# eliotwang/SageAttention

Measured on AMD Instinct MI355X. Metric: attention fwd TFLOPS at head_dim=128 seqlen=8192 (INT8 QK^T + FP16 PV, quantizers included), higher is better.
Workload: dtype int8+fp16; 1 GPU; c3: qk_int8_pv_fp16 (B,H,N,D)=(4,32,8192,128) causal=False qk_quant_gran=per_thread; global_batch=4, seq_len=8192, head_dim=128, heads=32, parallelism=single

## Files before the change

sageattention_amd/_build.py:

```python
import os
import subprocess
import sys

HERE = os.path.dirname(os.path.abspath(__file__))
CSRC = os.path.join(HERE, "csrc")
LIB = os.path.join(HERE, "libsageattn_hip.so")
HIPCC = os.environ.get("HIPCC", "/opt/rocm/bin/hipcc")
ARCH = "gfx950"

SOURCES = [
    ("sage_quant.hip", ["-ffp-contract=off"]),
    ("sage_attn.hip", ["-fno-slp-vectorize", "-ffp-contract=off"]),
    ("sage_fp8.hip", []),
    ("sage_misc.hip", []),
    ("sage_op.hip", []),
    ("sage_sparge.hip", []),
]
COMMON = ["-O3", "-std=c++17", "-fPIC", f"--offload-arch={ARCH}", "-Wall", "-Wno-unused-function", "-Wno-inline-asm",
          "-Rpass-analysis=kernel-resource-usage"]


def _check_no_scratch(src, compiler_output):
    import re
    name = None
    for line in compiler_output.splitlines():
        m = re.search(r"Function Name: (\S+)", line)
        if m:
            name = m.group(1)
        m = re.search(r"ScratchSize \[bytes/lane\]: (\d+)", line)
        if m and int(m.group(1)) != 0:
            raise RuntimeError(f"{src}: kernel {name} uses {m.group(1)} bytes/lane of scratch (register spill)")


def _check_occupancy(src, compiler_output):
    import re
    name = None
    for line in compiler_output.splitlines():
        m = re.search(r"Function Name: (\S+)", line)
        if m:
            name = m.group(1)
        m = re.search(r" VGPRs: (\d+)", line)
        guarded = name and (re.search(r"attn_i8_kernelILi64ELi4E(Lb[01]E){4}Lb0EEE", name) or
                            re.search(r"attn_i8_blocksparse_kernelILi64E(Lb[01]E){3}EE", name))
        if m and guarded and int(m.group(1)) > 168:
            raise RuntimeError(f"{src}: kernel {name} uses {m.group(1)} VGPRs (> 168: two waves per SIMD instead of three)")


def _check_m0_private(obj):
    import glob
    import re
    import shutil
    import tempfile
    objdump = os.path.join(os.path.dirname(os.path.dirname(HIPCC)), "lib", "llvm", "bin", "llvm-objdump")
    if not os.path.exists(objdump):
        objdump = "/opt/rocm/lib/llvm/bin/llvm-objdump"
    tmp = tempfile.mkdtemp(prefix="sage_m0_")
    try:
        local = os.path.join(tmp, "o.o")
        shutil.copy(obj, local)
        subprocess.run([objdump, "--offloading", local], stdout=subprocess.DEVNULL, stderr=subprocess.DEVNULL, check=True)
        dev = glob.glob(local + ".*" + ARCH)
        if not dev:
            raise RuntimeError(f"{obj}: no {ARCH} code object found")
        dis = subprocess.run([objdump, "-d", dev[0]], stdout=subprocess.PIPE, text=True, check=True).stdout
        bad = [l.strip() for l in dis.splitlines() if re.search(r"\bm0\b", l) and not re.search(r"s_mov_b32 m0, s\d+", l)]
        if bad:
            raise RuntimeError(f"{obj}: M0 is used outside lds_dma16:\n" + "\n".join(bad[:5]))
    finally:
        shutil.rmtree(tmp, ignore_errors=True)


def _digest(*parts) -> str:
    import hashlib
    h = hashlib.sha256()
    for part in parts:
        h.update(part if isinstance(part, bytes) else str(part).encode())
        h.update(b"\0")
    return h.hexdigest()


def _read(path) -> bytes:
    with open(path, "rb") as f:
        return f.read()


def _stamp_ok(target, key) -> bool:
    try:
        return os.path.exists(target) and _read(target + ".stamp").decode().strip() == key
    except OSError:
        return False


def _write_stamp(target, key):
    with open(target + ".stamp", "w") as f:
        f.write(key + "\n")


def build(force: bool = False, verbose: bool = False) -> str:
    hdrs = [os.path.join(CSRC, f) for f in sorted(os.listdir(CSRC)) if f.endswith(".h")]
    hdrs.append(os.path.join(HERE, "..", "include", "sageattn_hip.h"))
    hdr_key = _digest(*[_read(h) for h in hdrs])
    keys = {src: _digest(HIPCC, ARCH, " ".join(COMMON + extra), _read(os.path.join(CSRC, src)), hdr_key)
            for src, extra in SOURCES}
    lib_key = _digest(*[keys[src] for src, _ in SOURCES])
    if not force and _stamp_ok(LIB, lib_key):
        return LIB
    objs = []
    procs = []
    for src, extra in SOURCES:
        s = os.path.join(CSRC, src)
        o = os.path.join(CSRC, src.replace(".hip", ".o"))
        objs.append(o)
        if force or not _stamp_ok(o, keys[src]):
            cmd = [HIPCC] + COMMON + extra + ["-c", s, "-o", o]
            if verbose:
                print(" ".join(cmd), flush=True)
            procs.append((src, o, subprocess.Popen(cmd, stdout=subprocess.PIPE, stderr=subprocess.STDOUT, text=True)))
    for src, o, pr in procs:
        out, _ = pr.communicate()
        if pr.returncode != 0:
            raise RuntimeError(f"hipcc failed on {src}:\n{out}")
        try:
            _check_no_scratch(src, out)
            _check_occupancy(src, out)
        except RuntimeError:
            os.remove(o)
            raise
        _write_stamp(o, keys[src])
        if verbose:
            print("\n".join(l for l in out.splitlines() if "remark:" not in l))
    _check_m0_private(os.path.join(CSRC, "sage_attn.o"))
    cmd = [HIPCC, "-shared", "-fPIC", f"--offload-arch={ARCH}", "-o", LIB] + objs
    r = subprocess.run(cmd, stdout=subprocess.PIPE, stderr=subprocess.STDOUT, text=True)
    if r.returncode != 0:
        raise RuntimeError(f"link failed:\n{r.stdout}")
    _write_stamp(LIB, lib_key)
    return LIB


if __name__ == "__main__":
    print(build(force="--force" in sys.argv, verbose=True))
```

sageattention_amd/csrc/sage_quant.hip:

```cpp
#include "sage_entry.h"
#include "sage_fp8_kernels.h"

namespace sage {

constexpr int KMEAN_ROWS = 256;
__host__ __device__ __forceinline__ int kmean_chunk_rows(int N) {
  const int c256 = (N + KMEAN_ROWS - 1) / KMEAN_ROWS;
  return KMEAN_ROWS * ((c256 + 15) / 16 > 0 ? (c256 + 15) / 16 : 1);
}

template <int D, bool BF16>
__device__ __forceinline__ void k_mean_partial_body(const uint16_t* __restrict__ k, int64_t sb, int64_t sh, int64_t sn, int N,
                                                    float* __restrict__ part, int S, int s, int h, int b, int H,
                                                    float (*red)[D + 1]) {
  constexpr int TPR = D / 8;
  constexpr int RPP = 256 / TPR;
  const int tr = threadIdx.x / TPR, tc = threadIdx.x % TPR;
  const uint16_t* base = k + b * sb + h * sh + tc * 8;
  float acc[8] = {0, 0, 0, 0, 0, 0, 0, 0};
  const int rows = kmean_chunk_rows(N);
  const int r0 = s * rows;
  if (r0 + rows <= N) {
#pragma unroll 8
    for (int i = 0; i < rows / RPP; ++i) {
      const uint4 u = *reinterpret_cast<const uint4*>(base + (int64_t)(r0 + i * RPP + tr) * sn);
      float f[8];
      unpack8<BF16>(u, f);
#pragma unroll
      for (int j = 0; j < 8; ++j) acc[j] += f[j];
    }
  } else {
#pragma unroll 4
    for (int i = 0; i < rows / RPP; ++i) {
      const int row = r0 + i * RPP + tr;
      if (row < N) {
        const uint4 u = *reinterpret_cast<const uint4*>(base + (int64_t)row * sn);
        float f[8];
        unpack8<BF16>(u, f);
#pragma unroll
        for (int j = 0; j < 8; ++j) acc[j] += f[j];
      }
    }
  }
#pragma unroll
  for (int j = 0; j < 8; ++j) red[tr][tc * 8 + j] = acc[j];
  __syncthreads();
  if (threadIdx.x < D) {
    float sum = 0.f;
    for (int r = 0; r < RPP; ++r) sum += red[r][threadIdx.x];
    part[(((int64_t)b * H + h) * S + s) * D + threadIdx.x] = sum;
  }
}

template <int D, bool BF16>
__global__ __launch_bounds__(256) void k_mean_partial_kernel(const uint16_t* __restrict__ k, int64_t sb, int64_t sh,
                                                             int64_t sn, int N, float* __restrict__ part, int S) {
  __shared__ float red[256 / (D / 8)][D + 1];
  k_mean_partial_body<D, BF16>(k, sb, sh, sn, N, part, S, blockIdx.x, blockIdx.y, blockIdx.z, gridDim.y, red);
}

template <bool BF16>
__global__ void k_mean_final_kernel(const float* __restrict__ part, int S, int D, int N, uint16_t* __restrict__ km) {
  const int64_t bh = blockIdx.x;
  const int d = threadIdx.x;
  if (d >= D) return;
  float sum = 0.f;
  for (int s0 = 0; s0 < S; s0 += 8) {
    float v[8];
#pragma unroll
    for (int u = 0; u < 8; ++u) v[u] = part[(bh * S + min(s0 + u, S - 1)) * D + d];
#pragma unroll
    for (int u = 0; u < 8; ++u)
      if (s0 + u < S) sum += v[u];
  }
  km[bh * D + d] = f32_to_elem_bits<BF16>(sum / (float)N);
}


template <int CTRL>
__device__ __forceinline__ float dpp_lane(float x) {
  return __builtin_bit_cast(float, __builtin_amdgcn_update_dpp(0, __builtin_bit_cast(int, x), CTRL, 0xf, 0xf, false));
}
template <int TPR>
__device__ __forceinline__ float row_lanes_max(float a) {
  static_assert(TPR == 8 || TPR == 16, "a row is 8 or 16 lanes");
  a = fmaxf(a, dpp_lane<0xB1>(a));
  a = fmaxf(a, dpp_lane<0x4E>(a));
  a = fmaxf(a, dpp_lane<0x141>(a));
  if constexpr (TPR == 16) a = fmaxf(a, dpp_lane<0x140>(a));
  return a;
}

__device__ __forceinline__ int group_of_row(int lr, int gran, int is_key, int warp_shift) {
  if (gran == SAGE_GRAN_PER_BLOCK) return 0;
  const int w = lr >> warp_shift;
  if (gran == SAGE_GRAN_PER_WARP) return w;
  return is_key ? w * 4 + ((lr & 7) >> 1) : w * 8 + (lr & 7);
}

template <int D, int BLK>
struct QuantGeom {
  static constexpr int TPR = D / 8;
  static constexpr int RPP = 256 / TPR;
  static constexpr int NP = BLK / RPP;
  static_assert(NP >= 1, "block too small");
};

template <int D, int BLK>
__device__ __forceinline__ void quant_load_rows(const uint16_t* xbase, const int64_t xsn, const int blk, const int N_,
                                                uint4 (&raw)[QuantGeom<D, BLK>::NP]) {
  using G = QuantGeom<D, BLK>;
  int tid = threadIdx.x;
  asm volatile("" : "+v"(tid));
  const int tr = tid / G::TPR;
#pragma unroll
  for (int i = 0; i < G::NP; ++i) {
    const int row = blk * BLK + i * G::RPP + tr;
    raw[i] = make_uint4(0, 0, 0, 0);
    if (row < N_) raw[i] = *reinterpret_cast<const uint4*>(xbase + (int64_t)row * xsn);
  }
}

template <int D, bool BF16>
__device__ __forceinline__ uint4 quant_mean_bits(const QuantParams& p, const int h, const int b, const int H, const bool store_km,
                                                 float (*mpart)[D]) {
  constexpr int TPR = D / 8;
  const int tr = threadIdx.x / TPR, tc = threadIdx.x % TPR;
  if (p.mean_part && tr < p.S) {
    const float* pp = p.mean_part + (((int64_t)b * H + h) * p.S + tr) * D + tc * 8;
    *reinterpret_cast<float4*>(&mpart[tr][tc * 8]) = *reinterpret_cast<const float4*>(pp);
    *reinterpret_cast<float4*>(&mpart[tr][tc * 8 + 4]) = *reinterpret_cast<const float4*>(pp + 4);
  }
  __syncthreads();
  uint4 mbits = make_uint4(0u, 0u, 0u, 0u);
  if (p.mean_part) {
    if (tr == 0) {
      float sum[8] = {0, 0, 0, 0, 0, 0, 0, 0};
      for (int s_ = 0; s_ < p.S; ++s_) {
        const float4 a = *reinterpret_cast<const float4*>(&mpart[s_][tc * 8]), c = *reinterpret_cast<const float4*>(&mpart[s_][tc * 8 + 4]);
        sum[0] += a.x; sum[1] += a.y; sum[2] += a.z; sum[3] += a.w; sum[4] += c.x; sum[5] += c.y; sum[6] += c.z; sum[7] += c.w;
      }
      uint32_t w[4];
#pragma unroll
      for (int j = 0; j < 8; ++j) {
        const uint16_t bits = f32_to_elem_bits<BF16>(sum[j] / (float)p.N);
        if (j & 1) w[j >> 1] |= (uint32_t)bits << 16; else w[j >> 1] = bits;
      }
      mbits = make_uint4(w[0], w[1], w[2], w[3]);
      *reinterpret_cast<uint4*>(&mpart[0][tc * 8]) = mbits;
      if (store_km) *reinterpret_cast<uint4*>(p.km_out + ((int64_t)b * H + h) * D + tc * 8) = mbits;
    }
    __syncthreads();
    mbits = *reinterpret_cast<const uint4*>(&mpart[0][tc * 8]);
  } else if (p.mean) {
    mbits = *reinterpret_cast<const uint4*>(p.mean + ((int64_t)(p.cu ? 0 : b) * H + h) * D + tc * 8);
  }
  return mbits;
}

template <int D, int BLK, bool BF16, bool TRITON, typename AfterPhase1>
__device__ __forceinline__ void quant_block(const QuantParams& p, const int blk, const int h, const int b, const int H, const int N_,
                                            const int64_t o_boff, uint4 (&raw)[QuantGeom<D, BLK>::NP], const uint4 mbits,
                                            unsigned int* gmax, unsigned int* zero_next, AfterPhase1 after_phase1) {
  using G = QuantGeom<D, BLK>;
  constexpr int TPR = G::TPR, RPP = G::RPP, NP = G::NP;
  int tid = threadIdx.x;
  asm volatile("" : "+v"(tid));
  const int tr = tid / TPR, tc = tid % TPR;
  float xf[NP][8];
  float dvec[8];
  if (p.dot_vec) {
    const int Hk = H / p.dot_group;
    const uint4 ud = *reinterpret_cast<const uint4*>(p.dot_vec + ((int64_t)b * Hk + h / p.dot_group) * D + tc * 8);
    unpack8<BF16>(ud, dvec);
  }

  {
    float mean_f[8];
    if constexpr (!TRITON || BF16) unpack8<BF16>(mbits, mean_f);
#pragma unroll
    for (int i = 0; i < NP; ++i) {
      const int lr = i * RPP + tr;
      const int row = blk * BLK + lr;
      const bool valid = row < N_;
      if (p.dot_vec) {
        float xr[8];
        unpack8<BF16>(raw[i], xr);
        float dot = 0.f;
#pragma unroll
        for (int j = 0; j < 8; ++j) dot += xr[j] * dvec[j];
#pragma unroll
        for (int o = 1; o < TPR; o <<= 1) dot += __shfl_xor(dot, o);
        if (tc == 0 && valid) p.dot_out[((int64_t)b * H + h) * p.N + row] = dot;
      }
      if constexpr (TRITON && !BF16) {
        const uint32_t xw[4] = {raw[i].x, raw[i].y, raw[i].z, raw[i].w}, mw[4] = {mbits.x, mbits.y, mbits.z, mbits.w};
#pragma unroll
        for (int w = 0; w < 4; ++w) {
          const v2h d = __builtin_bit_cast(v2h, xw[w]) - __builtin_bit_cast(v2h, mw[w]);
          xf[i][2 * w] = (float)d[0];
          xf[i][2 * w + 1] = (float)d[1];
        }
      } else {
        unpack8<BF16>(raw[i], xf[i]);
#pragma unroll
        for (int j = 0; j < 8; ++j) {
          xf[i][j] = xf[i][j] - mean_f[j];
          if constexpr (TRITON) xf[i][j] = round_to_elem<BF16>(xf[i][j]);
        }
      }
      float amax = 0.f;
      const float mult_row = valid ? p.mult : 0.f;
#pragma unroll
      for (int j = 0; j < 8; ++j) {
        xf[i][j] = xf[i][j] * mult_row;
        amax = fmaxf(amax, fabsf(xf[i][j]));
      }
      amax = row_lanes_max<TPR>(amax);
      if (tc == 0) atomicMax(&gmax[group_of_row(lr, p.gran, p.is_key, p.warp_shift)], __float_as_uint(amax));
    }
  }
  after_phase1();
  __syncthreads();
  if (zero_next && threadIdx.x < 64) zero_next[threadIdx.x] = 0u;

  const int groups_per_blk = p.gran == SAGE_GRAN_PER_BLOCK ? 1
                             : p.gran == SAGE_GRAN_PER_WARP ? BLK >> p.warp_shift
                                                            : (BLK >> p.warp_shift) * (p.is_key ? 4 : 8);
  const float eps = (p.gran == SAGE_GRAN_PER_THREAD) ? 0.0000001f : 0.f;
  if (threadIdx.x < groups_per_blk) {
    const float a = __uint_as_float(gmax[threadIdx.x]);
    const float sc = TRITON ? a / 127.f + eps : fmaxf(a, 0.0000001f) / 127.f;
    p.scale[b * p.ss_b + h * p.ss_h + blk * p.ss_blk + threadIdx.x] = sc;
  }

  int8_t* obase = p.out + o_boff + h * p.osh + blk * p.o_blk + tc * 8;
#pragma unroll
  for (int i = 0; i < NP; ++i) {
    const int lr = i * RPP + tr;
    const int row = blk * BLK + lr;
    const float a = __uint_as_float(gmax[group_of_row(lr, p.gran, p.is_key, p.warp_shift)]);
    int q[8];
    if constexpr (TRITON) {
      const float sc = a / 127.f + eps;
      const float r = 1.0f / sc;
      bool near = false;
#pragma unroll
      for (int j = 0; j < 8; ++j) q[j] = round_half_away_fast(xf[i][j] * r, near);
      if (__builtin_amdgcn_ballot_w64(near || !(fabsf(r) < 3.0e38f)) != 0) {
#pragma unroll
        for (int j = 0; j < 8; ++j) {
          float y = xf[i][j] / sc;
          y = y + (y >= 0.f ? 0.5f : -0.5f);
          q[j] = min(max((int)y, -128), 127);
        }
      }
    } else {
      const float inv = 127.f / fmaxf(a, 0.0000001f);
#pragma unroll
      for (int j = 0; j < 8; ++j) q[j] = (int)rintf(xf[i][j] * inv);
    }
    const uint32_t w0 = pack_i8x4(q[0], q[1], q[2], q[3]), w1 = pack_i8x4(q[4], q[5], q[6], q[7]);
    if (row < N_) *reinterpret_cast<uint2*>(obase + (int64_t)lr * p.osn) = make_uint2(w0, w1);
  }
}

template <int D, int BLK, bool BF16, bool TRITON>
__device__ __forceinline__ void quant_qk_int8_body(const QuantParams& p, const int blk, const int h, const int b, const int H,
                                                   unsigned int* gmax, float (*mpart)[D]) {
  int N_ = p.N;
  int64_t x_boff = b * p.xsb, o_boff = b * p.osb;
  if (p.cu) {
    const int lo = p.cu[b];
    N_ = p.cu[b + 1] - lo;
    if (blk * BLK >= N_) return;
    x_boff = (int64_t)lo * p.xsn;
    o_boff = (int64_t)lo * p.osn;
  }
  if (threadIdx.x < 64) gmax[threadIdx.x] = 0u;
  uint4 raw[QuantGeom<D, BLK>::NP];
  quant_load_rows<D, BLK>(p.x + x_boff + h * p.xsh + (threadIdx.x % (D / 8)) * 8, p.xsn, blk, N_, raw);
  const uint4 mbits = quant_mean_bits<D, BF16>(p, h, b, H, blk == 0, mpart);
  quant_block<D, BLK, BF16, TRITON>(p, blk, h, b, H, N_, o_boff, raw, mbits, gmax, nullptr, [] {});
}

template <int D, int BLK, bool BF16, bool TRITON>
__global__ __launch_bounds__(256, BLK * D <= 64 * 128 ? 7 : 4) void quant_qk_int8_kernel(const QuantParams p) {
  __shared__ unsigned int gmax[64];
  __shared__ __attribute__((aligned(16))) float mpart[16][D];
  quant_qk_int8_body<D, BLK, BF16, TRITON>(p, blockIdx.x, blockIdx.y, blockIdx.z, gridDim.y, gmax, mpart);
}

template <int D, bool BF16, bool TRITON>
__device__ __forceinline__ void k_quant_stream_body(const QuantParams& p, const int per_wg, const int wg, const int h, const int b,
                                                    const int H, unsigned int (*gmax)[64], float (*mpart)[D]) {
  constexpr int BLK = 64;
  using G = QuantGeom<D, BLK>;
  const int nblk = (p.N + BLK - 1) / BLK;
  const int blk0 = wg * per_wg, blk1 = min(blk0 + per_wg, nblk);
  if (threadIdx.x < 192) (&gmax[0][0])[threadIdx.x] = 0u;
  const uint16_t* xbase = p.x + b * p.xsb + h * p.xsh + (threadIdx.x % G::TPR) * 8;
  const int64_t o_boff = b * p.osb;
  uint4 raw[G::NP];
  quant_load_rows<D, BLK>(xbase, p.xsn, blk0, p.N, raw);
  const uint4 mbits = quant_mean_bits<D, BF16>(p, h, b, H, wg == 0, mpart);
  int par = 0;
  for (int blk = blk0; blk < blk1; ++blk) {
    quant_block<D, BLK, BF16, TRITON>(p, blk, h, b, H, p.N, o_boff, raw, mbits, gmax[par], gmax[par == 0 ? 2 : par - 1], [&] {
      if (blk + 1 < blk1) quant_load_rows<D, BLK>(xbase, p.xsn, blk + 1, p.N, raw);
    });
    par = par == 2 ? 0 : par + 1;
  }
}

template <int D, bool BF16, bool TRITON>
__global__ __launch_bounds__(256, D == 64 ? 5 : 4) void k_quant_stream_kernel(const QuantParams p, const int per_wg) {
  __shared__ unsigned int gmax[3][64];
  __shared__ __attribute__((aligned(16))) float mpart[16][D];
  k_quant_stream_body<D, BF16, TRITON>(p, per_wg, blockIdx.x, blockIdx.y, blockIdx.z, gridDim.y, gmax, mpart);
}


template <int D, bool BF16>
__device__ __forceinline__ void v_amax_partial_body(const uint16_t* __restrict__ v, int64_t sb, int64_t sh, int64_t sn, int N,
                                                    float* __restrict__ part, int S, int s, int h, int b, int H,
                                                    float (*red)[D + 1]) {
  constexpr int TPR = D / 8, RPP = 256 / TPR;
  const int tr = threadIdx.x / TPR, tc = threadIdx.x % TPR;
  const uint16_t* base = v + b * sb + h * sh + tc * 8;
  float am[8] = {0, 0, 0, 0, 0, 0, 0, 0};
  const int rows = kmean_chunk_rows(N);
  if ((s + 1) * rows <= N) {
#pragma unroll 8
    for (int i = 0; i < rows / RPP; ++i) {
      float f[8];
      unpack8<BF16>(*reinterpret_cast<const uint4*>(base + (int64_t)(s * rows + i * RPP + tr) * sn), f);
#pragma unroll
      for (int j = 0; j < 8; ++j) am[j] = fmaxf(am[j], fabsf(f[j]));
    }
  } else {
#pragma unroll 4
    for (int i = 0; i < rows / RPP; ++i) {
      const int row = s * rows + i * RPP + tr;
      if (row < N) {
        float f[8];
        unpack8<BF16>(*reinterpret_cast<const uint4*>(base + (int64_t)row * sn), f);
#pragma unroll
        for (int j = 0; j < 8; ++j) am[j] = fmaxf(am[j], fabsf(f[j]));
      }
    }
  }
#pragma unroll
  for (int j = 0; j < 8; ++j) red[tr][tc * 8 + j] = am[j];
  __syncthreads();
  if (threadIdx.x < D) {
    float a = red[0][threadIdx.x];
    for (int r = 1; r < RPP; ++r) a = fmaxf(a, red[r][threadIdx.x]);
    part[(((int64_t)b * H + h) * S + s) * D + threadIdx.x] = a;
  }
}

template <int D, bool BF16>
__global__ __launch_bounds__(256) void kv_partial_kernel(const uint16_t* __restrict__ k, int64_t ksb, int64_t ksh, int64_t ksn,
                                                         const uint16_t* __restrict__ v, int64_t vsb, int64_t vsh, int64_t vsn,
                                                         int N, float* __restrict__ kpart, float* __restrict__ vpart, int S) {
  static_assert(KMEAN_ROWS == VQ_ROWS, "one chunk size for both tensors");
  __shared__ float red[256 / (D / 8)][D + 1];
  const int x = blockIdx.x;
  if (x < S) k_mean_partial_body<D, BF16>(k, ksb, ksh, ksn, N, kpart, S, x, blockIdx.y, blockIdx.z, gridDim.y, red);
  else v_amax_partial_body<D, BF16>(v, vsb, vsh, vsn, N, vpart, S, x - S, blockIdx.y, blockIdx.z, gridDim.y, red);
}

template <int D, bool BF16, bool TRITON>
__global__ __launch_bounds__(256, D == 64 ? 8 : 7) void kv_quant_kernel(const QuantParams p, const VPrepParams q, const int nblk_k) {
  using G = VQuantGeom<D>;
  __shared__ unsigned int gmax[64];
  __shared__ __attribute__((aligned(16))) float exch[16][D];
  __shared__ __attribute__((aligned(16))) uint32_t tile[G::BLKS * G::IMG];
  const int h = blockIdx.y, b = blockIdx.z, H = gridDim.y;
  if ((int)blockIdx.x < nblk_k) {
    quant_qk_int8_body<D, 64, BF16, TRITON>(p, blockIdx.x, h, b, H, gmax, exch);
    return;
  }
  const int bx = blockIdx.x - nblk_k;
  const int tg = threadIdx.x / G::TPR, tc = threadIdx.x % G::TPR;
  uint4 raw[4];
  v_quant_load<D>(q.v + b * q.sb + h * q.sh, q.sn, p.N, bx, raw);
  if (tg < p.S) {
    const float* pp = q.part + (((int64_t)b * H + h) * p.S + tg) * D + tc * 8;
    *reinterpret_cast<float4*>(&exch[tg][tc * 8]) = *reinterpret_cast<const float4*>(pp);
    *reinterpret_cast<float4*>(&exch[tg][tc * 8 + 4]) = *reinterpret_cast<const float4*>(pp + 4);
  }
  __syncthreads();
  if (tg == 0) {
    float rc[8], vs[8];
#pragma unroll
    for (int j = 0; j < 8; ++j) {
      float a = exch[0][tc * 8 + j];
      for (int s_ = 1; s_ < p.S; ++s_) a = fmaxf(a, exch[s_][tc * 8 + j]);
      rc[j] = q.scale_max / a;
      vs[j] = a / q.scale_max;
    }
#pragma unroll
    for (int j = 0; j < 8; ++j) exch[0][tc * 8 + j] = rc[j];
    if (bx == 0) {
      float* o = q.v_scale + ((int64_t)b * H + h) * D + tc * 8;
      *reinterpret_cast<float4*>(o) = make_float4(vs[0], vs[1], vs[2], vs[3]);
      *reinterpret_cast<float4*>(o + 4) = make_float4(vs[4], vs[5], vs[6], vs[7]);
    }
  }
  __syncthreads();
  float mean[8], rcp[8];
#pragma unroll
  for (int j = 0; j < 8; ++j) { mean[j] = 0.f; rcp[j] = exch[0][tc * 8 + j]; }
  v_quant_to_image<D, BF16>(raw, p.N, bx, mean, rcp, tile);
  __syncthreads();
  v_quant_store_image<D>(q.out, q.ob, q.oh, q.od, q.o_tile, p.N, bx, h, b, tile);
}

template <int D, bool BF16, bool TRITON>
__global__ __launch_bounds__(256, D == 64 ? 5 : 4) void kv_quant_stream_kernel(const QuantParams p, const VPrepParams q, const int per_k,
                                                                               const int nwg_k, const int per_v) {
  using G = VQuantGeom<D>;
  __shared__ unsigned int gmax[3][64];
  __shared__ __attribute__((aligned(16))) float exch[16][D];
  __shared__ __attribute__((aligned(16))) uint32_t tile[2][G::BLKS * G::IMG];
  const int h = blockIdx.y, b = blockIdx.z, H = gridDim.y;
  if ((int)blockIdx.x < nwg_k) {
    k_quant_stream_body<D, BF16, TRITON>(p, per_k, blockIdx.x, h, b, H, gmax, exch);
    return;
  }
  const int wg = blockIdx.x - nwg_k;
  const int nunits = ((p.N + 63) / 64 + G::BLKS - 1) / G::BLKS;
  const int u0 = wg * per_v, u1 = min(u0 + per_v, nunits);
  const uint16_t* vhead = q.v + b * q.sb + h * q.sh;
  uint4 raw[4];
  v_quant_load<D>(vhead, q.sn, p.N, u0, raw);
  const int tg = threadIdx.x / G::TPR, tc = threadIdx.x % G::TPR;
  if (tg < p.S) {
    const float* pp = q.part + (((int64_t)b * H + h) * p.S + tg) * D + tc * 8;
    *reinterpret_cast<float4*>(&exch[tg][tc * 8]) = *reinterpret_cast<const float4*>(pp);
    *reinterpret_cast<float4*>(&exch[tg][tc * 8 + 4]) = *reinterpret_cast<const float4*>(pp + 4);
  }
  __syncthreads();
  if (tg == 0) {
    float rc[8], vs[8];
#pragma unroll
    for (int j = 0; j < 8; ++j) {
      float a = exch[0][tc * 8 + j];
      for (int s_ = 1; s_ < p.S; ++s_) a = fmaxf(a, exch[s_][tc * 8 + j]);
      rc[j] = q.scale_max / a;
      vs[j] = a / q.scale_max;
    }
#pragma unroll
    for (int j = 0; j < 8; ++j) { exch[0][tc * 8 + j] = rc[j]; exch[1][tc * 8 + j] = vs[j]; }
    if (wg == 0) {
      float* o = q.v_scale + ((int64_t)b * H + h) * D + tc * 8;
      *reinterpret_cast<float4*>(o) = make_float4(vs[0], vs[1], vs[2], vs[3]);
      *reinterpret_cast<float4*>(o + 4) = make_float4(vs[4], vs[5], vs[6], vs[7]);
    }
  }
  __syncthreads();
  float mean[8], rcp[8];
#pragma unroll
  for (int j = 0; j < 8; ++j) { mean[j] = 0.f; rcp[j] = exch[0][tc * 8 + j]; }
  for (int u = u0; u < u1; ++u) {
    uint32_t* img = tile[(u - u0) & 1];
    v_quant_to_image<D, BF16>(raw, p.N, u, mean, rcp, img);
    if (u + 1 < u1) v_quant_load<D>(vhead, q.sn, p.N, u + 1, raw);
    __syncthreads();
    v_quant_store_image<D>(q.out, q.ob, q.oh, q.od, q.o_tile, p.N, u, h, b, img);
  }
}

template <bool BF16>
__global__ __launch_bounds__(256) void sub_mean_f16_kernel(const uint16_t* __restrict__ v, int64_t sb, int64_t sh,
                                                           int64_t sn, const uint16_t* __restrict__ vm,
                                                           uint16_t* __restrict__ out, int64_t ob, int64_t oh,
                                                           int64_t on, int N, int D) {
  const int TPR = D / 8, RPP = 256 / TPR;
  const int h = blockIdx.y, b = blockIdx.z, H = gridDim.y;
  const int tr = threadIdx.x / TPR, tc = threadIdx.x % TPR;
  const int row = blockIdx.x * RPP + tr;
  if (row >= N) return;
  float m[8], x[8];
  unpack8<BF16>(*reinterpret_cast<const uint4*>(vm + ((int64_t)b * H + h) * D + tc * 8), m);
  unpack8<BF16>(*reinterpret_cast<const uint4*>(v + b * sb + h * sh + (int64_t)row * sn + tc * 8), x);
  uint32_t w[4];
#pragma unroll
  for (int j = 0; j < 4; ++j) {
    const float lo = round_to_elem<BF16>(x[2 * j] - m[2 * j]);
    const float hi = round_to_elem<BF16>(x[2 * j + 1] - m[2 * j + 1]);
    w[j] = (uint32_t)f32_to_elem_bits<false>(lo) | ((uint32_t)f32_to_elem_bits<false>(hi) << 16);
  }
  *reinterpret_cast<uint4*>(out + b * ob + h * oh + (int64_t)row * on + tc * 8) = make_uint4(w[0], w[1], w[2], w[3]);
}


static int kmean_chunks(int N) {
  const int rows = kmean_chunk_rows(N);
  return (N + rows - 1) / rows;
}

static int units_per_wg(int64_t BH, int units, int64_t target, int64_t cap) {
  int64_t per = (BH * units + target - 1) / target;
  per = per > cap ? cap : per;
  return (int)(per < 1 ? 1 : per > units ? units : per);
}

static void launch_k_mean_partial(const sage_tensor& k, int B, int H, int N, int D, bool bf16, float* part, int S,
                                  hipStream_t st) {
  by_dim(D, [&](auto d) {
    by_flag(bf16, [&](auto bf) {
      hipLaunchKernelGGL((k_mean_partial_kernel<decltype(d)::value, decltype(bf)::value>), dim3(S, H, B), dim3(256), 0, st,
                         (const uint16_t*)k.data, k.stride_b, k.stride_h, k.stride_n, N, part, S);
    });
  });
}

int quant_check(QuantCall& c, const sage_tensor* x, int dtype, int B, int H, int N, int D, const void* mean,
                const sage_tensor* out, float* scale, int gran, int is_key, int blk, int warp, float mult, int rounding,
                const void* lse_dot_vec, int dot_group, float* lse_dot, const QuantOptions& opt) {
  if (!tensor_ok(x, 8) || !tensor_ok(out, 8) || !scale || B <= 0 || H <= 0 || N <= 0) return SAGE_ERR_INVALID_ARGUMENT;
  if (const int s = dim_dtype_status(D, dtype)) return s;
  if (gran < SAGE_GRAN_PER_BLOCK || gran > SAGE_GRAN_PER_THREAD) return SAGE_ERR_INVALID_ARGUMENT;
  if (rounding != SAGE_ROUND_TRITON && rounding != SAGE_ROUND_CUDA) return SAGE_ERR_INVALID_ARGUMENT;
  if (blk != 64 && blk != 128) return SAGE_ERR_INVALID_ARGUMENT;
  if (gran == SAGE_GRAN_PER_BLOCK) warp = blk;
  if ((warp != 16 && warp != 32 && warp != 64 && warp != 128) || blk % warp != 0) return SAGE_ERR_INVALID_ARGUMENT;
  if (mean && !aligned16(mean)) return SAGE_ERR_INVALID_ARGUMENT;
  if (opt.mean_part && (opt.S < 1 || opt.S > 16 || !aligned16(opt.mean_part))) return SAGE_ERR_INVALID_ARGUMENT;
  if ((lse_dot_vec != nullptr) != (lse_dot != nullptr)) return SAGE_ERR_INVALID_ARGUMENT;
  if (lse_dot_vec && (dot_group <= 0 || H % dot_group != 0 || !aligned16(lse_dot_vec))) return SAGE_ERR_INVALID_ARGUMENT;
  const int nblk = (N + blk - 1) / blk;
  const int gpb = gran == SAGE_GRAN_PER_BLOCK ? 1 : gran == SAGE_GRAN_PER_WARP ? blk / warp : (blk / warp) * (is_key ? 4 : 8);
  if (gpb > 64) return SAGE_ERR_INVALID_ARGUMENT;
  QuantParams& p = c.p;
  p.x = (const uint16_t*)x->data; p.xsb = x->stride_b; p.xsh = x->stride_h; p.xsn = x->stride_n;
  p.mean = (const uint16_t*)mean;
  p.out = (int8_t*)out->data; p.osb = out->stride_b; p.osh = out->stride_h; p.osn = out->stride_n;
  p.scale = scale; p.dot_vec = (const uint16_t*)lse_dot_vec; p.dot_out = lse_dot; p.dot_group = dot_group > 0 ? dot_group : 1;
  p.cu = opt.cu;
  p.mean_part = opt.mean_part; p.S = opt.S; p.km_out = (uint16_t*)opt.km_out;
  p.o_blk = opt.out_blk_stride ? opt.out_blk_stride : (int64_t)blk * out->stride_n;
  p.ss_b = opt.scale_strides ? opt.scale_strides[0] : (int64_t)H * nblk * gpb;
  p.ss_h = opt.scale_strides ? opt.scale_strides[1] : (int64_t)nblk * gpb;
  p.ss_blk = opt.scale_strides ? opt.scale_strides[2] : gpb;
  if (opt.out_blk_stride < 0 || (opt.out_blk_stride & 7) || p.ss_blk < gpb) return SAGE_ERR_INVALID_ARGUMENT;
  p.N = N; p.G = nblk * gpb; p.gran = gran; p.is_key = is_key ? 1 : 0; p.warp = warp; p.mult = mult; p.rounding = rounding;
  p.warp_shift = warp == 16 ? 4 : warp == 32 ? 5 : warp == 64 ? 6 : 7;
  c.B = B; c.H = H; c.D = D; c.blk = blk; c.bf16 = dtype == SAGE_BF16;
  return SAGE_OK;
}

int quant_launch(const QuantCall& c, hipStream_t st) {
  const dim3 grid((c.p.N + c.blk - 1) / c.blk, c.H, c.B);
  launch_begin();
  by_dim(c.D, [&](auto d) {
    by_flag(c.blk == 128, [&](auto b128) {
      by_flag(c.bf16, [&](auto bf) {
        by_flag(c.p.rounding == SAGE_ROUND_TRITON, [&](auto tr) {
          constexpr int BLK = decltype(b128)::value ? 128 : 64;
          hipLaunchKernelGGL((quant_qk_int8_kernel<decltype(d)::value, BLK, decltype(bf)::value, decltype(tr)::value>), grid,
                             dim3(256), 0, st, c.p);
        });
      });
    });
  });
  return launch_status();
}

int k_smooth_quant_check(KSmoothCall& c, const sage_tensor* k, int dtype, int B, int H, int N, int D, const sage_tensor* out,
                         float* scale, void* km, int gran, int rounding, void* workspace) {
  if (!km || !workspace) return SAGE_ERR_INVALID_ARGUMENT;
  if (gran != SAGE_GRAN_PER_BLOCK && gran != SAGE_GRAN_PER_THREAD) return SAGE_ERR_INVALID_ARGUMENT;
  if (!tensor_ok(k, 8) || B <= 0 || H <= 0 || N <= 0) return SAGE_ERR_INVALID_ARGUMENT;
  if (const int s = dim_dtype_status(D, dtype)) return s;
  QuantOptions opt;
  opt.mean_part = c.part = (float*)workspace;
  opt.S = kmean_chunks(N);
  opt.km_out = km;
  if (const int s = quant_check(c.q, k, dtype, B, H, N, D, nullptr, out, scale, gran, 1, 64, 64, 1.0f, rounding, nullptr, 1,
                                nullptr, opt))
    return s;
  c.k = *k;
  const int nblk = (N + 63) / 64;
  c.per_wg = units_per_wg((int64_t)B * H, nblk, 256 * (D == 64 ? 5 : 4), nblk);
  return SAGE_OK;
}

int k_smooth_quant_launch(const KSmoothCall& c, hipStream_t st) {
  const QuantParams& p = c.q.p;
  launch_begin();
  launch_k_mean_partial(c.k, c.q.B, c.q.H, p.N, c.q.D, c.q.bf16, c.part, p.S, st);
  if (launch_status() != SAGE_OK) return SAGE_ERR_LAUNCH;
  const int nblk = (p.N + 63) / 64;
  const dim3 grid((nblk + c.per_wg - 1) / c.per_wg, c.q.H, c.q.B);
  launch_begin();
  by_dim(c.q.D, [&](auto d) {
    by_flag(c.q.bf16, [&](auto bf) {
      by_flag(p.rounding == SAGE_ROUND_TRITON, [&](auto tr) {
        hipLaunchKernelGGL((k_quant_stream_kernel<decltype(d)::value, decltype(bf)::value, decltype(tr)::value>), grid,
                           dim3(256), 0, st, p, c.per_wg);
      });
    });
  });
  return launch_status();
}

int kv_prepare_check(KVPrepCall& c, const sage_tensor* k, const sage_tensor* v, int dtype, int B, int H, int N, int D,
                     const sage_tensor* k_int8, float* k_scale, void* km, int gran, int rounding, const sage_tensor* v_fp8,
                     float* v_scale, float scale_max, void* workspace) {
  if (!km || !workspace || !v_scale || !(scale_max > 0.f)) return SAGE_ERR_INVALID_ARGUMENT;
  if (gran != SAGE_GRAN_PER_BLOCK && gran != SAGE_GRAN_PER_THREAD) return SAGE_ERR_INVALID_ARGUMENT;
  if (!tensor_ok(k, 8) || !tensor_ok(v, 8) || B <= 0 || H <= 0 || N <= 0) return SAGE_ERR_INVALID_ARGUMENT;
  if (!tensor_ok(v_fp8, 16)) return SAGE_ERR_INVALID_ARGUMENT;
  if (const int s = dim_dtype_status(D, dtype)) return s;
  const int S = kmean_chunks(N);
  c.kpart = (float*)workspace;
  c.vpart = c.kpart + (size_t)B * H * S * D;
  QuantOptions opt;
  opt.mean_part = c.kpart;
  opt.S = S;
  opt.km_out = km;
  if (const int s = quant_check(c.k, k, dtype, B, H, N, D, nullptr, k_int8, k_scale, gran, 1, 64, 64, 1.0f, rounding, nullptr,
                                1, nullptr, opt))
    return s;
  VPrepParams& q = c.v;
  q.v = (const uint16_t*)v->data; q.sb = v->stride_b; q.sh = v->stride_h; q.sn = v->stride_n;
  q.out = (uint8_t*)v_fp8->data; q.ob = v_fp8->stride_b; q.oh = v_fp8->stride_h; q.od = v_fp8->stride_n; q.o_tile = 64;
  q.v_scale = v_scale; q.part = c.vpart; q.scale_max = scale_max;
  c.nblk_k = (N + 63) / 64;
  const int blks = by_dim(D, [](auto d) { return VQuantGeom<decltype(d)::value>::BLKS; });
  c.nunit_v = (c.nblk_k + blks - 1) / blks;
  const int64_t target = 128 * (D == 64 ? 5 : 4), cap = 32;
  c.per_k = units_per_wg((int64_t)B * H, c.nblk_k, target, cap);
  c.per_v = units_per_wg((int64_t)B * H, c.nunit_v, target, cap);
  c.streaming = c.per_v >= (D == 64 ? 4 : 12);
  return SAGE_OK;
}

int kv_prepare_launch(const KVPrepCall& c, hipStream_t st) {
  const QuantParams& p = c.k.p;
  const VPrepParams& q = c.v;
  const int B = c.k.B, H = c.k.H;
  launch_begin();
  by_dim(c.k.D, [&](auto d) {
    by_flag(c.k.bf16, [&](auto bf) {
      hipLaunchKernelGGL((kv_partial_kernel<decltype(d)::value, decltype(bf)::value>), dim3(2 * p.S, H, B), dim3(256), 0, st,
                         p.x, p.xsb, p.xsh, p.xsn, q.v, q.sb, q.sh, q.sn, p.N, c.kpart, c.vpart, p.S);
    });
  });
  if (launch_status() != SAGE_OK) return SAGE_ERR_LAUNCH;
  const int nwg_k = (c.nblk_k + c.per_k - 1) / c.per_k, nwg_v = (c.nunit_v + c.per_v - 1) / c.per_v;
  by_dim(c.k.D, [&](auto d) {
    by_flag(c.k.bf16, [&](auto bf) {
      by_flag(p.rounding == SAGE_ROUND_TRITON, [&](auto tr) {
        constexpr int DD = decltype(d)::value;
        constexpr bool BF = decltype(bf)::value, TR = decltype(tr)::value;
        if (c.streaming)
          hipLaunchKernelGGL((kv_quant_stream_kernel<DD, BF, TR>), dim3(nwg_k + nwg_v, H, B), dim3(256), 0, st, p, q, c.per_k,
                             nwg_k, c.per_v);
        else
          hipLaunchKernelGGL((kv_quant_kernel<DD, BF, TR>), dim3(c.nblk_k + c.nunit_v, H, B), dim3(256), 0, st, p, q, c.nblk_k);
      });
    });
  });
  return launch_status();
}

}

using namespace sage;

extern "C" size_t sage_k_mean_workspace_bytes(int B, int H, int N, int D) {
  const size_t S = (size_t)(N + KMEAN_ROWS - 1) / KMEAN_ROWS;
  return (size_t)B * H * S * D * sizeof(float);
}

extern "C" int sage_k_mean(const sage_tensor* k, int dtype, int B, int H, int N, int D, void* km, void* workspace,
                           sage_stream_t stream) {
  if (!tensor_ok(k, 8) || !km || !workspace || B <= 0 || H <= 0 || N <= 0) return SAGE_ERR_INVALID_ARGUMENT;
  if (const int s = dim_dtype_status(D, dtype)) return s;
  const int S = kmean_chunks(N);
  float* const ws = (float*)workspace;
  hipStream_t st = (hipStream_t)stream;
  launch_begin();
  launch_k_mean_partial(*k, B, H, N, D, dtype == SAGE_BF16, ws, S, st);
  by_flag(dtype == SAGE_BF16, [&](auto bf) {
    hipLaunchKernelGGL((k_mean_final_kernel<decltype(bf)::value>), dim3(B * H), dim3(128), 0, st, ws, S, D, N, (uint16_t*)km);
  });
  return launch_status();
}

extern "C" int sage_quant_qk_int8(const sage_tensor* x, int dtype, int B, int H, int N, int D, const void* mean,
                                  const sage_tensor* out, float* scale, int gran, int is_key, int blk, int warp,
                                  float mult, int rounding, const void* lse_dot_vec, int dot_group, float* lse_dot,
                                  sage_stream_t stream) {
  QuantCall c;
  if (const int s = quant_check(c, x, dtype, B, H, N, D, mean, out, scale, gran, is_key, blk, warp, mult, rounding,
                                lse_dot_vec, dot_group, lse_dot))
    return s;
  return quant_launch(c, (hipStream_t)stream);
}

extern "C" int sage_quant_qk_int8_varlen(const sage_tensor* x, int dtype, const int* cu_seqlens, int num_seqs, int H,
                                         int max_seqlen, int D, const void* mean, const sage_tensor* out, float* scale,
                                         int gran, int is_key, int blk, int warp, float mult, int rounding,
                                         sage_stream_t stream) {
  if (!cu_seqlens) return SAGE_ERR_INVALID_ARGUMENT;
  QuantOptions opt;
  opt.cu = cu_seqlens;
  QuantCall c;
  if (const int s = quant_check(c, x, dtype, num_seqs, H, max_seqlen, D, mean, out, scale, gran, is_key, blk, warp, mult,
                                rounding, nullptr, 1, nullptr, opt))
    return s;
  return quant_launch(c, (hipStream_t)stream);
}

extern "C" int sage_sub_mean_f16(const sage_tensor* v, int dtype, int B, int H, int N, int D, const void* vm,
                                 const sage_tensor* out, sage_stream_t stream) {
  if (!tensor_ok(v, 8) || !tensor_ok(out, 8) || !vm || !aligned16(vm) || B <= 0 || H <= 0 || N <= 0) return SAGE_ERR_INVALID_ARGUMENT;
  if (const int s = dim_dtype_status(D, dtype)) return s;
  const int RPP = 256 / (D / 8);
  const dim3 grid((N + RPP - 1) / RPP, H, B);
  launch_begin();
  by_flag(dtype == SAGE_BF16, [&](auto bf) {
    hipLaunchKernelGGL((sub_mean_f16_kernel<decltype(bf)::value>), grid, dim3(256), 0, (hipStream_t)stream,
                       (const uint16_t*)v->data, v->stride_b, v->stride_h, v->stride_n, (const uint16_t*)vm,
                       (uint16_t*)out->data, out->stride_b, out->stride_h, out->stride_n, N, D);
  });
  return launch_status();
}

extern "C" int sage_quant_k_int8_kvtiles(const sage_tensor* k, int dtype, int B, int H, int N, int D, const void* mean,
                                         const sage_tensor* out, int64_t out_tile_stride, float* scale,
                                         const int64_t* scale_strides, int gran, int rounding, sage_stream_t stream) {
  if (!scale_strides || out_tile_stride <= 0) return SAGE_ERR_INVALID_ARGUMENT;
  if (gran != SAGE_GRAN_PER_BLOCK && gran != SAGE_GRAN_PER_THREAD) return SAGE_ERR_INVALID_ARGUMENT;
  QuantOptions opt;
  opt.out_blk_stride = out_tile_stride;
  opt.scale_strides = scale_strides;
  QuantCall c;
  if (const int s = quant_check(c, k, dtype, B, H, N, D, mean, out, scale, gran, 1, 64, 64, 1.0f, rounding, nullptr, 1, nullptr,
                                opt))
    return s;
  return quant_launch(c, (hipStream_t)stream);
}

extern "C" int sage_k_smooth_quant(const sage_tensor* k, int dtype, int B, int H, int N, int D, const sage_tensor* out,
                                   float* scale, void* km, int gran, int rounding, void* workspace, sage_stream_t stream) {
  KSmoothCall c;
  if (const int s = k_smooth_quant_check(c, k, dtype, B, H, N, D, out, scale, km, gran, rounding, workspace)) return s;
  return k_smooth_quant_launch(c, (hipStream_t)stream);
}

extern "C" size_t sage_kv_prepare_fp8_workspace_bytes(int B, int H, int N, int D) {
  return sage_k_mean_workspace_bytes(B, H, N, D) + sage_quant_v_fp8_workspace_bytes(B, H, N, D);
}

extern "C" int sage_kv_prepare_fp8(const sage_tensor* k, const sage_tensor* v, int dtype, int B, int H, int N, int D,
                                   const sage_tensor* k_int8, float* k_scale, void* km, int gran, int rounding,
                                   const sage_tensor* v_fp8, float* v_scale, float scale_max, void* workspace,
                                   sage_stream_t stream) {
  KVPrepCall c;
  if (const int s = kv_prepare_check(c, k, v, dtype, B, H, N, D, k_int8, k_scale, km, gran, rounding, v_fp8, v_scale,
                                     scale_max, workspace))
    return s;
  return kv_prepare_launch(c, (hipStream_t)stream);
}
```

Measured before the change: 1325 TFLOPS.

## Specialize streaming K quantizer per granularity with single-atomic amax and magic rounding

Adds a dedicated K-quant block routine for the streaming kernel, specialized at compile time for per-thread versus other granularities and for full versus ragged tail blocks. Each thread now reduces amax across all its rows before doing one atomic, instead of one per row. Rounding uses a magic-number FMA with a wave-wide ballot fallback to exact division. The DPP row max now works on uint bits and SLP vectorization is disabled for the quant file. The aim is to cut quantizer ALU, atomic and branch overhead. The cost is more template instantiations and code size, plus the need for the fast rounding path to match the reference exactly.

```diff
diff --git a/sageattention_amd/_build.py b/sageattention_amd/_build.py
--- a/sageattention_amd/_build.py
+++ b/sageattention_amd/_build.py
@@ -9,7 +9,7 @@
 ARCH = "gfx950"
 
 SOURCES = [
-    ("sage_quant.hip", ["-ffp-contract=off"]),
+    ("sage_quant.hip", ["-fno-slp-vectorize", "-ffp-contract=off"]),
     ("sage_attn.hip", ["-fno-slp-vectorize", "-ffp-contract=off"]),
     ("sage_fp8.hip", []),
     ("sage_misc.hip", []),
diff --git a/sageattention_amd/csrc/sage_quant.hip b/sageattention_amd/csrc/sage_quant.hip
--- a/sageattention_amd/csrc/sage_quant.hip
+++ b/sageattention_amd/csrc/sage_quant.hip
@@ -78,17 +78,18 @@
 
 
 template <int CTRL>
-__device__ __forceinline__ float dpp_lane(float x) {
-  return __builtin_bit_cast(float, __builtin_amdgcn_update_dpp(0, __builtin_bit_cast(int, x), CTRL, 0xf, 0xf, false));
+__device__ __forceinline__ unsigned int dpp_max_u32(unsigned int x) {
+  return max(x, (unsigned int)__builtin_amdgcn_update_dpp((int)x, (int)x, CTRL, 0xf, 0xf, true));
 }
 template <int TPR>
 __device__ __forceinline__ float row_lanes_max(float a) {
   static_assert(TPR == 8 || TPR == 16, "a row is 8 or 16 lanes");
-  a = fmaxf(a, dpp_lane<0xB1>(a));
-  a = fmaxf(a, dpp_lane<0x4E>(a));
-  a = fmaxf(a, dpp_lane<0x141>(a));
-  if constexpr (TPR == 16) a = fmaxf(a, dpp_lane<0x140>(a));
-  return a;
+  unsigned int u = __float_as_uint(a);
+  u = dpp_max_u32<0xB1>(u);
+  u = dpp_max_u32<0x4E>(u);
+  u = dpp_max_u32<0x141>(u);
+  if constexpr (TPR == 16) u = dpp_max_u32<0x140>(u);
+  return __uint_as_float(u);
 }
 
 __device__ __forceinline__ int group_of_row(int lr, int gran, int is_key, int warp_shift) {
@@ -158,10 +159,30 @@
   return mbits;
 }
 
-template <int D, int BLK, bool BF16, bool TRITON, typename AfterPhase1>
+template <bool BF16, bool TRITON>
+__device__ __forceinline__ void sub_mean8(const uint4& raw, const uint4& mbits, const float (&mean_f)[8], float (&xf)[8]) {
+  if constexpr (TRITON && !BF16) {
+    const uint32_t xw[4] = {raw.x, raw.y, raw.z, raw.w}, mw[4] = {mbits.x, mbits.y, mbits.z, mbits.w};
+#pragma unroll
+    for (int w = 0; w < 4; ++w) {
+      const v2h d = __builtin_bit_cast(v2h, xw[w]) - __builtin_bit_cast(v2h, mw[w]);
+      xf[2 * w] = (float)d[0];
+      xf[2 * w + 1] = (float)d[1];
+    }
+  } else {
+    unpack8<BF16>(raw, xf);
+#pragma unroll
+    for (int j = 0; j < 8; ++j) {
+      xf[j] = xf[j] - mean_f[j];
+      if constexpr (TRITON) xf[j] = round_to_elem<BF16>(xf[j]);
+    }
+  }
+}
+
+template <int D, int BLK, bool BF16, bool TRITON>
 __device__ __forceinline__ void quant_block(const QuantParams& p, const int blk, const int h, const int b, const int H, const int N_,
                                             const int64_t o_boff, uint4 (&raw)[QuantGeom<D, BLK>::NP], const uint4 mbits,
-                                            unsigned int* gmax, unsigned int* zero_next, AfterPhase1 after_phase1) {
+                                            unsigned int* gmax) {
   using G = QuantGeom<D, BLK>;
   constexpr int TPR = G::TPR, RPP = G::RPP, NP = G::NP;
   int tid = threadIdx.x;
@@ -193,22 +214,7 @@
         for (int o = 1; o < TPR; o <<= 1) dot += __shfl_xor(dot, o);
         if (tc == 0 && valid) p.dot_out[((int64_t)b * H + h) * p.N + row] = dot;
       }
-      if constexpr (TRITON && !BF16) {
-        const uint32_t xw[4] = {raw[i].x, raw[i].y, raw[i].z, raw[i].w}, mw[4] = {mbits.x, mbits.y, mbits.z, mbits.w};
-#pragma unroll
-        for (int w = 0; w < 4; ++w) {
-          const v2h d = __builtin_bit_cast(v2h, xw[w]) - __builtin_bit_cast(v2h, mw[w]);
-          xf[i][2 * w] = (float)d[0];
-          xf[i][2 * w + 1] = (float)d[1];
-        }
-      } else {
-        unpack8<BF16>(raw[i], xf[i]);
-#pragma unroll
-        for (int j = 0; j < 8; ++j) {
-          xf[i][j] = xf[i][j] - mean_f[j];
-          if constexpr (TRITON) xf[i][j] = round_to_elem<BF16>(xf[i][j]);
-        }
-      }
+      sub_mean8<BF16, TRITON>(raw[i], mbits, mean_f, xf[i]);
       float amax = 0.f;
       const float mult_row = valid ? p.mult : 0.f;
 #pragma unroll
@@ -220,9 +226,7 @@
       if (tc == 0) atomicMax(&gmax[group_of_row(lr, p.gran, p.is_key, p.warp_shift)], __float_as_uint(amax));
     }
   }
-  after_phase1();
-  __syncthreads();
-  if (zero_next && threadIdx.x < 64) zero_next[threadIdx.x] = 0u;
+  __syncthreads();
 
   const int groups_per_blk = p.gran == SAGE_GRAN_PER_BLOCK ? 1
                              : p.gran == SAGE_GRAN_PER_WARP ? BLK >> p.warp_shift
@@ -281,7 +285,7 @@
   uint4 raw[QuantGeom<D, BLK>::NP];
   quant_load_rows<D, BLK>(p.x + x_boff + h * p.xsh + (threadIdx.x % (D / 8)) * 8, p.xsn, blk, N_, raw);
   const uint4 mbits = quant_mean_bits<D, BF16>(p, h, b, H, blk == 0, mpart);
-  quant_block<D, BLK, BF16, TRITON>(p, blk, h, b, H, N_, o_boff, raw, mbits, gmax, nullptr, [] {});
+  quant_block<D, BLK, BF16, TRITON>(p, blk, h, b, H, N_, o_boff, raw, mbits, gmax);
 }
 
 template <int D, int BLK, bool BF16, bool TRITON>
@@ -291,26 +295,136 @@
   quant_qk_int8_body<D, BLK, BF16, TRITON>(p, blockIdx.x, blockIdx.y, blockIdx.z, gridDim.y, gmax, mpart);
 }
 
+
+template <int D, bool CLAMP>
+__device__ __forceinline__ void k_load_rows(const uint16_t* xbase, const int64_t xsn, const int blk, const int N,
+                                            uint4 (&raw)[QuantGeom<D, 64>::NP]) {
+  using G = QuantGeom<D, 64>;
+  const int row0 = blk * 64 + (int)threadIdx.x / G::TPR;
+#pragma unroll
+  for (int i = 0; i < G::NP; ++i) {
+    const int row = CLAMP ? min(row0 + i * G::RPP, N - 1) : row0 + i * G::RPP;
+    raw[i] = *reinterpret_cast<const uint4*>(xbase + (int64_t)row * xsn);
+  }
+}
+
+__device__ __forceinline__ uint2 round_half_away_pack8(const float (&x)[8], const float r, bool& near) {
+  constexpr float M = 12582912.f;
+  uint32_t tb[8];
+  float res[8];
+#pragma unroll
+  for (int j = 0; j < 8; ++j) {
+    const float t = __builtin_fmaf(x[j], r, M);
+    res[j] = __builtin_fmaf(x[j], r, -(t - M));
+    tb[j] = __float_as_uint(t);
+  }
+  float m = fmaxf(fmaxf(fabsf(res[0]), fabsf(res[1])), fabsf(res[2]));
+  m = fmaxf(fmaxf(m, fabsf(res[3])), fabsf(res[4]));
+  m = fmaxf(fmaxf(m, fabsf(res[5])), fabsf(res[6]));
+  m = fmaxf(m, fabsf(res[7]));
+  near = !(m <= 0.5f - 6.1035156e-5f);
+  return make_uint2(pack_i8x4(tb[0], tb[1], tb[2], tb[3]), pack_i8x4(tb[4], tb[5], tb[6], tb[7]));
+}
+
+template <int D, bool BF16, bool TRITON, bool PER_THREAD, bool RAGGED, typename AfterPhase1>
+__device__ __forceinline__ void k_quant_block(const QuantParams& p, const int blk, const int h, const int b,
+                                              uint4 (&raw)[QuantGeom<D, 64>::NP], const uint4 mbits, unsigned int* gmax,
+                                              unsigned int* zero_next, AfterPhase1 after_phase1) {
+  using G = QuantGeom<D, 64>;
+  constexpr int TPR = G::TPR, RPP = G::RPP, NP = G::NP, NG = PER_THREAD ? 4 : 1;
+  static_assert(RPP % 8 == 0, "the group of a row must not depend on the pass");
+  const int tr = (int)threadIdx.x / TPR, tc = (int)threadIdx.x % TPR;
+  const int g = PER_THREAD ? (tr & 7) >> 1 : 0;
+  const int row0 = blk * 64 + tr;
+  float xf[NP][8];
+  {
+    float mean_f[8];
+    if constexpr (!TRITON || BF16) unpack8<BF16>(mbits, mean_f);
+    float amax = 0.f;
+#pragma unroll
+    for (int i = 0; i < NP; ++i) {
+      sub_mean8<BF16, TRITON>(raw[i], mbits, mean_f, xf[i]);
+      float am = RAGGED ? 0.f : amax;
+#pragma unroll
+      for (int j = 0; j < 8; ++j) am = fmaxf(am, fabsf(xf[i][j]));
+      if constexpr (RAGGED) amax = fmaxf(amax, row0 + i * RPP < p.N ? am : 0.f);
+      else amax = am;
+    }
+    amax = row_lanes_max<TPR>(amax);
+    if (tc == 0) atomicMax(&gmax[g], __float_as_uint(amax));
+  }
+  after_phase1();
+  __syncthreads();
+  if (threadIdx.x < NG) zero_next[threadIdx.x] = 0u;
+
+  const float a = __uint_as_float(gmax[g]);
+  const float sc = TRITON ? a / 127.f + (PER_THREAD ? 0.0000001f : 0.f) : 0.f;
+  const float r = TRITON ? 1.0f / sc : 127.f / fmaxf(a, 0.0000001f);
+  if (tc == 0 && tr < 2 * NG && !(tr & 1))
+    p.scale[b * p.ss_b + h * p.ss_h + blk * p.ss_blk + g] = TRITON ? sc : fmaxf(a, 0.0000001f) / 127.f;
+  const bool r_unusable = TRITON && !(fabsf(r) < 3.0e38f);
+
+  int8_t* obase = p.out + b * p.osb + h * p.osh + blk * p.o_blk + (int64_t)tr * p.osn + tc * 8;
+#pragma unroll
+  for (int i = 0; i < NP; ++i) {
+    uint2 w;
+    if constexpr (TRITON) {
+      bool near;
+      w = round_half_away_pack8(xf[i], r, near);
+      if (__builtin_amdgcn_ballot_w64(near || r_unusable) != 0) {
+        int q[8];
+#pragma unroll
+        for (int j = 0; j < 8; ++j) {
+          float y = xf[i][j] / sc;
+          y = y + (y >= 0.f ? 0.5f : -0.5f);
+          q[j] = min(max((int)y, -128), 127);
+        }
+        w = make_uint2(pack_i8x4(q[0], q[1], q[2], q[3]), pack_i8x4(q[4], q[5], q[6], q[7]));
+      }
+    } else {
+      uint32_t tb[8];
+#pragma unroll
+      for (int j = 0; j < 8; ++j) tb[j] = __float_as_uint(xf[i][j] * r + 12582912.f);
+      w = make_uint2(pack_i8x4(tb[0], tb[1], tb[2], tb[3]), pack_i8x4(tb[4], tb[5], tb[6], tb[7]));
+    }
+    if (!RAGGED || row0 + i * RPP < p.N) *reinterpret_cast<uint2*>(obase + (int64_t)(i * RPP) * p.osn) = w;
+  }
+}
+
+template <int D, bool BF16, bool TRITON, bool PER_THREAD>
+__device__ __forceinline__ void k_quant_stream_walk(const QuantParams& p, const int per_wg, const int wg, const int h, const int b,
+                                                    const int H, unsigned int (*gmax)[64], float (*mpart)[D]) {
+  using G = QuantGeom<D, 64>;
+  const int nblk = (p.N + 63) / 64, nfull = p.N / 64;
+  const int blk0 = wg * per_wg, blk1 = min(blk0 + per_wg, nblk);
+  if (threadIdx.x < 192) (&gmax[0][0])[threadIdx.x] = 0u;
+  const uint16_t* xbase = p.x + b * p.xsb + h * p.xsh + (threadIdx.x % G::TPR) * 8;
+  uint4 raw[G::NP];
+  if (blk0 < nfull) k_load_rows<D, false>(xbase, p.xsn, blk0, p.N, raw);
+  else k_load_rows<D, true>(xbase, p.xsn, blk0, p.N, raw);
+  const uint4 mbits = quant_mean_bits<D, BF16>(p, h, b, H, wg == 0, mpart);
+  int par = 0;
+  for (int blk = blk0; blk < blk1; ++blk) {
+    unsigned int* const zero_next = gmax[par == 0 ? 2 : par - 1];
+    if (blk < nfull) {
+      k_quant_block<D, BF16, TRITON, PER_THREAD, false>(p, blk, h, b, raw, mbits, gmax[par], zero_next, [&] {
+        if (blk + 1 < blk1) {
+          if (blk + 1 < nfull) k_load_rows<D, false>(xbase, p.xsn, blk + 1, p.N, raw);
+          else k_load_rows<D, true>(xbase, p.xsn, blk + 1, p.N, raw);
+        }
+      });
+    } else {
+      k_quant_block<D, BF16, TRITON, PER_THREAD, true>(p, blk, h, b, raw, mbits, gmax[par], zero_next, [] {});
+    }
+    par = par == 2 ? 0 : par + 1;
+  }
+}
+
 template <int D, bool BF16, bool TRITON>
 __device__ __forceinline__ void k_quant_stream_body(const QuantParams& p, const int per_wg, const int wg, const int h, const int b,
                                                     const int H, unsigned int (*gmax)[64], float (*mpart)[D]) {
-  constexpr int BLK = 64;
-  using G = QuantGeom<D, BLK>;
-  const int nblk = (p.N + BLK - 1) / BLK;
-  const int blk0 = wg * per_wg, blk1 = min(blk0 + per_wg, nblk);
-  if (threadIdx.x < 192) (&gmax[0][0])[threadIdx.x] = 0u;
-  const uint16_t* xbase = p.x + b * p.xsb + h * p.xsh + (threadIdx.x % G::TPR) * 8;
-  const int64_t o_boff = b * p.osb;
-  uint4 raw[G::NP];
-  quant_load_rows<D, BLK>(xbase, p.xsn, blk0, p.N, raw);
-  const uint4 mbits = quant_mean_bits<D, BF16>(p, h, b, H, wg == 0, mpart);
-  int par = 0;
-  for (int blk = blk0; blk < blk1; ++blk) {
-    quant_block<D, BLK, BF16, TRITON>(p, blk, h, b, H, p.N, o_boff, raw, mbits, gmax[par], gmax[par == 0 ? 2 : par - 1], [&] {
-      if (blk + 1 < blk1) quant_load_rows<D, BLK>(xbase, p.xsn, blk + 1, p.N, raw);
-    });
-    par = par == 2 ? 0 : par + 1;
-  }
+  if (p.gran == SAGE_GRAN_PER_THREAD) k_quant_stream_walk<D, BF16, TRITON, true>(p, per_wg, wg, h, b, H, gmax, mpart);
+  else k_quant_stream_walk<D, BF16, TRITON, false>(p, per_wg, wg, h, b, H, gmax, mpart);
 }
 
 template <int D, bool BF16, bool TRITON>
```

New measurement: 1340 TFLOPS, median of 6. +1.2%, better.
